# thierrydumas/autoencoder_based_image_compression

Hardware: AMD Instinct MI355X
Metric: Mpixels/s encode+decode (Kodak 768x512 luma), bitstream bit-exact (higher is better)
Workload: dtype f32; 1 GPU; kodak_512x768_luma_batch24_per_gpu_bin_width_1.0_lossless_roundtrip; height=512, width=768, truncated_unary_length=10, idx_map_exception=67, parallelism=single GPU, coder=device, 64 maps per wavefront, encode + decode + compare

## Files before the change

### autoencoder_based_image_compression_amd/csrc/hip/conv_gemm_split.hip

```cpp
#include "conv_gemm.h"

#include <cstdlib>

using namespace eae_conv_gemm;

namespace {

constexpr int RING = 8;
#ifndef EAE_EPI_RING
#define EAE_EPI_RING 4
#endif
constexpr int EPI_RING = EAE_EPI_RING;
constexpr int ABUF = 32 * AS_STRIDE;
constexpr int vec_floats(int norm) { return (norm >= NORM_LATENT ? 5 : 2) * EAE_C; }
constexpr int QT_H = 4, QT_W = 8;
constexpr int MIN_PIECE = 4;
constexpr int SPIN_LIMIT = 1 << 22;

__device__ __forceinline__ int head_steps(int d, int D, int T) {
    return T < 3 * MIN_PIECE ? T : MIN_PIECE + (d * (T - 2 * MIN_PIECE)) / D;
}

template <int NORM, int WPB>
__global__ __launch_bounds__(64 * WPB, NORM >= NORM_LATENT ? 2 : 3) void conv_gemm_split_kernel(const ConvGemmParams p) {
    __shared__ __attribute__((aligned(16))) float lds[WPB * 2 * ABUF + vec_floats(NORM)];
#ifdef EAE_GEMM_PRIO
    __builtin_amdgcn_s_setprio(EAE_GEMM_PRIO);
#endif
    const int lane = threadIdx.x & 63;
    const int wave = __builtin_amdgcn_readfirstlane(threadIdx.x >> 6);
    float* wlds = lds + wave * 2 * ABUF;
    float* vec_lds = lds + WPB * 2 * ABUF;
    {
        const float2 z = make_float2(0.f, 0.f);
        *reinterpret_cast<float2*>(vec_lds + 2 * lane) = p.bias ? *reinterpret_cast<const float2*>(p.bias + 2 * lane) : z;
        if (NORM == EAE_NORM_GDN || NORM == EAE_NORM_IGDN || NORM == NORM_LATENT)
            *reinterpret_cast<float2*>(vec_lds + EAE_C + 2 * lane) = *reinterpret_cast<const float2*>(p.beta + 2 * lane);
        if (NORM >= NORM_LATENT) {
            if (NORM == NORM_LATENT_PLAIN) *reinterpret_cast<float2*>(vec_lds + EAE_C + 2 * lane) = z;
            *reinterpret_cast<float2*>(vec_lds + 2 * EAE_C + 2 * lane) = NORM == NORM_LATENT ? *reinterpret_cast<const float2*>(p.beta_out + 2 * lane) : z;
            *reinterpret_cast<float2*>(vec_lds + 3 * EAE_C + 2 * lane) = p.map_mean ? *reinterpret_cast<const float2*>(p.map_mean + 2 * lane) : z;
            *reinterpret_cast<float2*>(vec_lds + 4 * EAE_C + 2 * lane) = *reinterpret_cast<const float2*>(p.bin_widths + 2 * lane);
        }
    }
    const int hi = lane >> 5, lj = lane & 31, a_q = lane & 7;
    const int cbase = 4 * hi;

    const int x = (int)blockIdx.x & 7;
    const int wx = p.split_resident_waves_per_xcd;
    const int nsp = p.n * p.tiles_r * p.tiles_c;
    const int q8 = nsp >> 3, r8 = nsp & 7;
    const int cnt_sp = q8 + (x < r8 ? 1 : 0);
    const int first_sp = x * q8 + (x < r8 ? x : r8);
    const int ntt = cnt_sp * p.n_phases;
    const int D = p.split ? (ntt < wx ? ntt : wx) : 0;
    const int F = ntt - D;
    const int n_items = 2 * D + F;
    unsigned int* flags = p.split_ws + 256 + x * 1024;

    const __amdgpu_buffer_rsrc_t w_rsrc = __builtin_amdgcn_make_buffer_rsrc(
        const_cast<float*>(p.w), 0, (int)((size_t)MAX_TAPS * EAE_C * EAE_C * sizeof(float)), 0x00020000);
    const int w_lane = (hi * EAE_C + lj * 4) * 4;
    const int a_off = lj * AS_STRIDE + hi * 16;

    {
        const int item = ((int)blockIdx.x >> 3) * WPB + wave;
        if (item >= n_items) return;
        int d = -1, tau;
        bool is_tail = false;
        if (item < D) { d = item; tau = ntt - D + d; }
        else if (item < D + F) { tau = item - D; }
        else { d = item - D - F; tau = ntt - D + d; is_tail = true; }
        int ph = 0, sp = tau;
        while (sp >= cnt_sp) { sp -= cnt_sp; ++ph; }
        const PhaseDesc& pd = p.phase[ph];
        const int ntaps = pd.ntaps;
        const int tap_of_lane = pd.tap[lane < MAX_TAPS ? lane : 0];
#define EAE_Q_TAP(ti_) __builtin_amdgcn_readlane(tap_of_lane, (ti_))
        const int T = (EAE_C / KC) * ntaps;
        int s0 = 0, s1 = T;
        if (d >= 0) {
            const int h = head_steps(d, D, T);
            if (is_tail) { if (h >= T) return; s0 = h; }
            else s1 = h;
        }
        int b = first_sp + sp;
        const int tc = b % p.tiles_c; b /= p.tiles_c;
        const int tr = b % p.tiles_r;
        const int img = b / p.tiles_r;

        int a_pr[4], a_pc[4], a_ok[4];
        const int a_m0 = 4 * ((lane >> 3) & 3) + 16 * (lane >> 5);
#pragma unroll
        for (int i = 0; i < 4; ++i) {
            const int m = a_m0 + i;
            a_pr[i] = tr * QT_H + m / QT_W;
            a_pc[i] = tc * QT_W + m % QT_W;
            a_ok[i] = (a_pr[i] < p.hp) & (a_pc[i] < p.wp);
        }
        const float* in_img = p.in + (size_t)img * p.hin * p.win * EAE_C;
        const __amdgpu_buffer_rsrc_t in_rsrc = __builtin_amdgcn_make_buffer_rsrc(
            const_cast<float*>(in_img), 0, (int)((size_t)p.hin * p.win * EAE_C * sizeof(float)), 0x00020000);
        const int pr = tr * QT_H + lj / QT_W, pc = tc * QT_W + lj % QT_W;
        const bool valid = pr < p.hp && pc < p.wp;
        float* out_img = p.out + (size_t)img * p.hout * p.wout * EAE_C;
        const int o_off = ((pr * p.out_stride + pd.out_a) * p.wout + (pc * p.out_stride + pd.out_b)) * EAE_C;
        float* o = out_img + o_off;
        const __amdgpu_buffer_rsrc_t out_rsrc = __builtin_amdgcn_make_buffer_rsrc(
            out_img, 0, (int)((size_t)p.hout * p.wout * EAE_C * sizeof(float)), 0x00020000);
        const int park = valid ? (o_off + cbase) * 4 : -1;

        float4 a_reg[4];
#define EAE_Q_PREFETCH_A(packed_, ci0_)                                                                              \
        {                                                                                                            \
            const int dr_ = ((packed_) & 0xFF) - 8, dc_ = (((packed_) >> 8) & 0xFF) - 8;                             \
            _Pragma("unroll") for (int i = 0; i < 4; ++i) {                                                          \
                const int r_ = a_pr[i] * p.in_stride + dr_;                                                          \
                const int c_ = a_pc[i] * p.in_stride + dc_;                                                          \
                const int ok_ = a_ok[i] & ((unsigned)r_ < (unsigned)p.hin) & ((unsigned)c_ < (unsigned)p.win);       \
                const int lin_ = ((r_ * p.win + c_) * EAE_C + (ci0_) + 4 * a_q) * 4;                                 \
                const u32x4 v_ = __builtin_amdgcn_raw_buffer_load_b128(in_rsrc, ok_ ? lin_ : -1, 0, 0);              \
                a_reg[i] = make_float4(__uint_as_float(v_.x), __uint_as_float(v_.y), __uint_as_float(v_.z),          \
                                       __uint_as_float(v_.w));                                                       \
            }                                                                                                        \
        }
#define EAE_Q_STAGE_A(buf_)                                                                                          \
        {                                                                                                            \
            _Pragma("unroll") for (int i = 0; i < 4; ++i) {                                                          \
                float* dst_ = wlds + (buf_) * ABUF + (a_m0 + i) * AS_STRIDE + 2 * a_q;                              \
                *reinterpret_cast<float2*>(dst_) = make_float2(a_reg[i].x, a_reg[i].z);                              \
                *reinterpret_cast<float2*>(dst_ + 16) = make_float2(a_reg[i].y, a_reg[i].w);                         \
            }                                                                                                        \
        }
#define EAE_Q_SLAB(ti_, ch_) ((((EAE_Q_TAP(ti_) >> 16) * EAE_C + (ch_) * KC) * EAE_C) * 4)
#define EAE_Q_W_LOAD(dst_, slab_, kk_)                                                                               \
        {                                                                                                            \
            const u32x4 v_ = __builtin_amdgcn_raw_buffer_load_b128(w_rsrc, w_lane + (kk_) * 2 * EAE_C * 4, (slab_), 0); \
            dst_ = make_float4(__uint_as_float(v_.x), __uint_as_float(v_.y), __uint_as_float(v_.z),                  \
                               __uint_as_float(v_.w));                                                               \
        }

        f32x16 acc[4];
        if (s0 == 0) {
#pragma unroll
            for (int t = 0; t < 4; ++t)
#pragma unroll
                for (int r = 0; r < 16; ++r) acc[t][r] = 0.f;
        } else {
            int gave_up = 0;
            if (lane == 0) {
                int spins = 0;
                while (__hip_atomic_load(flags + d, __ATOMIC_RELAXED, __HIP_MEMORY_SCOPE_AGENT) == 0u) {
                    __builtin_amdgcn_s_sleep(8);
                    if (++spins > p.split_spin_limit) { gave_up = 1; break; }
                }
            }
            if (__builtin_amdgcn_readfirstlane(gave_up)) {
                if (lane == 0) atomicAdd(p.split_ws + SPLIT_ERROR_WORD, 1u);
                return;
            }
            __builtin_amdgcn_wave_barrier();
            asm volatile("" ::: "memory");
#pragma unroll
            for (int t = 0; t < 4; ++t)
#pragma unroll
                for (int g = 0; g < 4; ++g) {
                    const u32x4 v = __builtin_amdgcn_raw_buffer_load_b128(out_rsrc, park, (32 * t + 8 * g) * 4, 16);
                    acc[t][4 * g + 0] = __uint_as_float(v.x); acc[t][4 * g + 1] = __uint_as_float(v.y);
                    acc[t][4 * g + 2] = __uint_as_float(v.z); acc[t][4 * g + 3] = __uint_as_float(v.w);
                }
            if (lane == 0) __hip_atomic_store(flags + d, 0u, __ATOMIC_RELAXED, __HIP_MEMORY_SCOPE_AGENT);
        }

        int tap_i = s0 % ntaps, chunk = s0 / ntaps;
        float4 ring[RING];
        {
            const int slab0 = EAE_Q_SLAB(tap_i, chunk);
#pragma unroll
            for (int i = 0; i < RING; ++i) EAE_Q_W_LOAD(ring[i], slab0, i)
        }
        EAE_Q_PREFETCH_A(EAE_Q_TAP(tap_i), chunk * KC)
        EAE_Q_STAGE_A(0)
        for (int step = s0; step < s1; ++step) {
            int nti = tap_i + 1, nch = chunk;
            if (nti == ntaps) { nti = 0; ++nch; }
            if (step + 1 >= s1) { nti = tap_i; nch = chunk; }
            const int slab_cur = EAE_Q_SLAB(tap_i, chunk);
            const int slab_nxt = EAE_Q_SLAB(nti, nch);
            EAE_Q_PREFETCH_A(EAE_Q_TAP(nti), nch * KC)
            const float4* a_rd = reinterpret_cast<const float4*>(wlds + ((step - s0) & 1) * ABUF + a_off);
            const float4 a0 = a_rd[0], a1 = a_rd[1], a2 = a_rd[2], a3 = a_rd[3];
            const float av[16] = {a0.x, a0.y, a0.z, a0.w, a1.x, a1.y, a1.z, a1.w, a2.x, a2.y, a2.z, a2.w, a3.x, a3.y, a3.z, a3.w};
            __builtin_amdgcn_sched_barrier(0);
#pragma unroll
            for (int kk = 0; kk < KC / 2; ++kk) {
                const float4 wq = ring[kk % RING];
                acc[0] = mfma32(wq.x, av[kk], acc[0]);
                acc[1] = mfma32(wq.y, av[kk], acc[1]);
                acc[2] = mfma32(wq.z, av[kk], acc[2]);
                acc[3] = mfma32(wq.w, av[kk], acc[3]);
                if (kk + RING < KC / 2) { EAE_Q_W_LOAD(ring[kk % RING], slab_cur, kk + RING) }
                else { EAE_Q_W_LOAD(ring[kk % RING], slab_nxt, kk + RING - KC / 2) }
                __builtin_amdgcn_sched_group_barrier(0x008, 4, 0);
                __builtin_amdgcn_sched_group_barrier(0x020, 1, 0);
            }
            __builtin_amdgcn_sched_barrier(0);
            EAE_Q_STAGE_A(((step - s0) + 1) & 1)
            tap_i = nti;
            chunk = nch;
        }

        if (s1 == T) {
            if constexpr (NORM >= NORM_LATENT) {
                if (p.bias) {
#pragma unroll
                    for (int t = 0; t < 4; ++t)
#pragma unroll
                        for (int g = 0; g < 4; ++g) {
                            const float4 bv = *reinterpret_cast<const float4*>(vec_lds + 32 * t + 8 * g + cbase);
                            acc[t][4 * g + 0] = acc[t][4 * g + 0] + bv.x;
                            acc[t][4 * g + 1] = acc[t][4 * g + 1] + bv.y;
                            acc[t][4 * g + 2] = acc[t][4 * g + 2] + bv.z;
                            acc[t][4 * g + 3] = acc[t][4 * g + 3] + bv.w;
                        }
                }
                wave_latent_body<NORM == NORM_LATENT, NORM == NORM_LATENT>(acc, vec_lds + EAE_C, p.gamma, p.gamma_out, p.latent, valid,
                                                                           (long)img, pr * p.wp + pc, p.hp * p.wp, lane);
            } else {
                wave_epilogue<NORM, EPI_RING>(acc, vec_lds, p.bias != nullptr, p.gamma, o, valid, lane);
            }
        } else {
#pragma unroll
            for (int t = 0; t < 4; ++t)
#pragma unroll
                for (int g = 0; g < 4; ++g) {
                    const u32x4 v = {__float_as_uint(acc[t][4 * g]), __float_as_uint(acc[t][4 * g + 1]),
                                     __float_as_uint(acc[t][4 * g + 2]), __float_as_uint(acc[t][4 * g + 3])};
                    __builtin_amdgcn_raw_buffer_store_b128(v, out_rsrc, park, (32 * t + 8 * g) * 4, 16);
                }
            asm volatile("s_waitcnt vmcnt(0)" ::: "memory");
            if (lane == 0 && !p.split_mute_heads) __hip_atomic_store(flags + d, 1u, __ATOMIC_RELAXED, __HIP_MEMORY_SCOPE_AGENT);
        }
#undef EAE_Q_PREFETCH_A
#undef EAE_Q_STAGE_A
#undef EAE_Q_SLAB
#undef EAE_Q_TAP
#undef EAE_Q_W_LOAD
    }
}

}

int eae_conv_gemm::launch_split(ConvGemmParams& p, hipStream_t stream, int cut) {
    const int cus = eae_compute_units();
    if (cus < 8 || (cus & 7)) return 1;
    p.tiles_r = (p.hp + QT_H - 1) / QT_H;
    p.tiles_c = (p.wp + QT_W - 1) / QT_W;
    const long nsp = (long)p.n * p.tiles_r * p.tiles_c;
    const long tiles = nsp * p.n_phases;
    const long simds = 4L * cus;
    long k = tiles / simds;
    if (k > 3) k = 3;
    if (k < 1) k = 1;
    const bool validated = eae_is_whole_mi355x();
    bool split = cut > 0;
    if (cut > 0) k = cut > 3 ? 3 : cut;
    if (cut < 0 && validated && p.split_ws && p.n_phases == 1 && tiles >= simds) {
        const long rounds = (tiles + simds - 1) / simds;
        split = (double)rounds * simds > 1.03 * (double)tiles || tiles >= 3 * simds;
    }
    if (split && !p.split_ws) return EAE_HIP_BAD_ARGUMENT;
    if (p.norm >= NORM_LATENT && k > 2) k = 2;
    if ((cus / 8) * 4 * k > 1024) return 1;
    for (int i = 1; i < p.n_phases; ++i)
        for (int j = i; j > 0 && p.phase[j].ntaps > p.phase[j - 1].ntaps; --j) {
            const PhaseDesc tmp = p.phase[j]; p.phase[j] = p.phase[j - 1]; p.phase[j - 1] = tmp;
        }
    p.split = split ? 1 : 0;
    p.split_spin_limit = SPIN_LIMIT;
    p.split_mute_heads = 0;
    if (split) {
        if (g_eae_launch_options.split_mute) { p.split_mute_heads = 1; p.split_spin_limit = 1 << 12; }
    }
    p.split_resident_waves_per_xcd = (cus / 8) * 4 * (int)k;
    const long cnt_max = (nsp + 7) / 8 * p.n_phases;
    const long d_max = split ? (cnt_max < p.split_resident_waves_per_xcd ? cnt_max : p.split_resident_waves_per_xcd) : 0;
    const int wpb = g_eae_launch_options.split_wpb == 1 ? 1 : 4;
    const int grid = (int)((cnt_max + d_max + wpb - 1) / wpb) * 8;
#define EAE_LAUNCH_S(N_)                                                                                                  \
    {                                                                                                                     \
        if (wpb == 1) hipLaunchKernelGGL((conv_gemm_split_kernel<N_, 1>), dim3(grid), dim3(64), 0, stream, p);            \
        else hipLaunchKernelGGL((conv_gemm_split_kernel<N_, 4>), dim3(grid), dim3(256), 0, stream, p);                    \
    }
    if (p.norm == NORM_LATENT) EAE_LAUNCH_S(NORM_LATENT)
    else if (p.norm == NORM_LATENT_PLAIN) EAE_LAUNCH_S(NORM_LATENT_PLAIN)
    else if (p.norm == EAE_NORM_GDN) EAE_LAUNCH_S(EAE_NORM_GDN)
    else if (p.norm == EAE_NORM_IGDN) EAE_LAUNCH_S(EAE_NORM_IGDN)
    else EAE_LAUNCH_S(EAE_NORM_NONE)
#undef EAE_LAUNCH_S
    EAE_HIP_CHECK_LAUNCH();
    return EAE_HIP_OK;
}
```

Measured before the change: 2976 Mpixels/s.

## Simplify A-tile staging with padded single LDS buffer and precomputed tap masks

Replaces the double-buffered, swizzled A-tile LDS staging with one buffer per wave using a KC+1 padded row stride. Each lane now loads its own output pixel's channels, and the per-element LDS reads are stride-2. Address math is simplified: a per-lane base offset plus a bitmask of out-of-bounds taps, computed once per work item, replace the per-prefetch row/column bounds checks. The aims are to cut VALU address arithmetic and LDS footprint. The cost is 16 scalar LDS reads and scalar writes per step instead of vector ones, and reliance on in-order LDS access within a wave for the single buffer.

Measured after the change: 3026 Mpixels/s, median of 6. +1.7%, better.

```diff
diff --git a/autoencoder_based_image_compression_amd/csrc/hip/conv_gemm_split.hip b/autoencoder_based_image_compression_amd/csrc/hip/conv_gemm_split.hip
--- a/autoencoder_based_image_compression_amd/csrc/hip/conv_gemm_split.hip
+++ b/autoencoder_based_image_compression_amd/csrc/hip/conv_gemm_split.hip
@@ -11,7 +11,8 @@
 #define EAE_EPI_RING 4
 #endif
 constexpr int EPI_RING = EAE_EPI_RING;
-constexpr int ABUF = 32 * AS_STRIDE;
+constexpr int A_STRIDE = KC + 1;
+constexpr int ABUF = 32 * A_STRIDE;
 constexpr int vec_floats(int norm) { return (norm >= NORM_LATENT ? 5 : 2) * EAE_C; }
 constexpr int QT_H = 4, QT_W = 8;
 constexpr int MIN_PIECE = 4;
@@ -23,14 +24,14 @@
 
 template <int NORM, int WPB>
 __global__ __launch_bounds__(64 * WPB, NORM >= NORM_LATENT ? 2 : 3) void conv_gemm_split_kernel(const ConvGemmParams p) {
-    __shared__ __attribute__((aligned(16))) float lds[WPB * 2 * ABUF + vec_floats(NORM)];
+    __shared__ __attribute__((aligned(16))) float lds[WPB * ABUF + vec_floats(NORM)];
 #ifdef EAE_GEMM_PRIO
     __builtin_amdgcn_s_setprio(EAE_GEMM_PRIO);
 #endif
     const int lane = threadIdx.x & 63;
     const int wave = __builtin_amdgcn_readfirstlane(threadIdx.x >> 6);
-    float* wlds = lds + wave * 2 * ABUF;
-    float* vec_lds = lds + WPB * 2 * ABUF;
+    float* wlds = lds + wave * ABUF;
+    float* vec_lds = lds + WPB * ABUF;
     {
         const float2 z = make_float2(0.f, 0.f);
         *reinterpret_cast<float2*>(vec_lds + 2 * lane) = p.bias ? *reinterpret_cast<const float2*>(p.bias + 2 * lane) : z;
@@ -43,7 +44,7 @@
             *reinterpret_cast<float2*>(vec_lds + 4 * EAE_C + 2 * lane) = *reinterpret_cast<const float2*>(p.bin_widths + 2 * lane);
         }
     }
-    const int hi = lane >> 5, lj = lane & 31, a_q = lane & 7;
+    const int hi = lane >> 5, lj = lane & 31;
     const int cbase = 4 * hi;
 
     const int x = (int)blockIdx.x & 7;
@@ -61,7 +62,6 @@
     const __amdgpu_buffer_rsrc_t w_rsrc = __builtin_amdgcn_make_buffer_rsrc(
         const_cast<float*>(p.w), 0, (int)((size_t)MAX_TAPS * EAE_C * EAE_C * sizeof(float)), 0x00020000);
     const int w_lane = (hi * EAE_C + lj * 4) * 4;
-    const int a_off = lj * AS_STRIDE + hi * 16;
 
     {
         const int item = ((int)blockIdx.x >> 3) * WPB + wave;
@@ -89,18 +89,6 @@
         const int tr = b % p.tiles_r;
         const int img = b / p.tiles_r;
 
-        int a_pr[4], a_pc[4], a_ok[4];
-        const int a_m0 = 4 * ((lane >> 3) & 3) + 16 * (lane >> 5);
-#pragma unroll
-        for (int i = 0; i < 4; ++i) {
-            const int m = a_m0 + i;
-            a_pr[i] = tr * QT_H + m / QT_W;
-            a_pc[i] = tc * QT_W + m % QT_W;
-            a_ok[i] = (a_pr[i] < p.hp) & (a_pc[i] < p.wp);
-        }
-        const float* in_img = p.in + (size_t)img * p.hin * p.win * EAE_C;
-        const __amdgpu_buffer_rsrc_t in_rsrc = __builtin_amdgcn_make_buffer_rsrc(
-            const_cast<float*>(in_img), 0, (int)((size_t)p.hin * p.win * EAE_C * sizeof(float)), 0x00020000);
         const int pr = tr * QT_H + lj / QT_W, pc = tc * QT_W + lj % QT_W;
         const bool valid = pr < p.hp && pc < p.wp;
         float* out_img = p.out + (size_t)img * p.hout * p.wout * EAE_C;
@@ -110,29 +98,38 @@
             out_img, 0, (int)((size_t)p.hout * p.wout * EAE_C * sizeof(float)), 0x00020000);
         const int park = valid ? (o_off + cbase) * 4 : -1;
 
+        const float* in_img = p.in + (size_t)img * p.hin * p.win * EAE_C;
+        const __amdgpu_buffer_rsrc_t in_rsrc = __builtin_amdgcn_make_buffer_rsrc(
+            const_cast<float*>(in_img), 0, (int)((size_t)p.hin * p.win * EAE_C * sizeof(float)), 0x00020000);
+        const int a_r = pr * p.in_stride, a_c = pc * p.in_stride;
+        const unsigned int a_base = ((unsigned)a_r * (unsigned)p.win + (unsigned)a_c) * (EAE_C * 4) + 16 * hi;
+        unsigned int a_inv = 0;
+        for (int ti = 0; ti < ntaps; ++ti) {
+            const int packed = EAE_Q_TAP(ti);
+            const int r = a_r + (packed & 0xFF) - 8, c = a_c + ((packed >> 8) & 0xFF) - 8;
+            if (!valid || (unsigned)r >= (unsigned)p.hin || (unsigned)c >= (unsigned)p.win) a_inv |= 1u << ti;
+        }
+
         float4 a_reg[4];
-#define EAE_Q_PREFETCH_A(packed_, ci0_)                                                                              \
+#define EAE_Q_PREFETCH_A(packed_, ti_, ci0_)                                                                         \
         {                                                                                                            \
             const int dr_ = ((packed_) & 0xFF) - 8, dc_ = (((packed_) >> 8) & 0xFF) - 8;                             \
+            const unsigned int off_ = (a_base + (unsigned)(((dr_ * p.win + dc_) * EAE_C + (ci0_)) * 4)) |            \
+                                      ((a_inv >> (ti_)) << 31);                                                      \
             _Pragma("unroll") for (int i = 0; i < 4; ++i) {                                                          \
-                const int r_ = a_pr[i] * p.in_stride + dr_;                                                          \
-                const int c_ = a_pc[i] * p.in_stride + dc_;                                                          \
-                const int ok_ = a_ok[i] & ((unsigned)r_ < (unsigned)p.hin) & ((unsigned)c_ < (unsigned)p.win);       \
-                const int lin_ = ((r_ * p.win + c_) * EAE_C + (ci0_) + 4 * a_q) * 4;                                 \
-                const u32x4 v_ = __builtin_amdgcn_raw_buffer_load_b128(in_rsrc, ok_ ? lin_ : -1, 0, 0);              \
+                const u32x4 v_ = __builtin_amdgcn_raw_buffer_load_b128(in_rsrc, (int)off_ + 32 * i, 0, 0);           \
                 a_reg[i] = make_float4(__uint_as_float(v_.x), __uint_as_float(v_.y), __uint_as_float(v_.z),          \
                                        __uint_as_float(v_.w));                                                       \
             }                                                                                                        \
         }
-#define EAE_Q_STAGE_A(buf_)                                                                                          \
+#define EAE_Q_STAGE_A()                                                                                              \
         {                                                                                                            \
             _Pragma("unroll") for (int i = 0; i < 4; ++i) {                                                          \
-                float* dst_ = wlds + (buf_) * ABUF + (a_m0 + i) * AS_STRIDE + 2 * a_q;                              \
-                *reinterpret_cast<float2*>(dst_) = make_float2(a_reg[i].x, a_reg[i].z);                              \
-                *reinterpret_cast<float2*>(dst_ + 16) = make_float2(a_reg[i].y, a_reg[i].w);                         \
+                float* dst_ = wlds + lj * A_STRIDE + 8 * i + 4 * hi;                                                 \
+                dst_[0] = a_reg[i].x; dst_[1] = a_reg[i].y; dst_[2] = a_reg[i].z; dst_[3] = a_reg[i].w;              \
             }                                                                                                        \
         }
-#define EAE_Q_SLAB(ti_, ch_) ((((EAE_Q_TAP(ti_) >> 16) * EAE_C + (ch_) * KC) * EAE_C) * 4)
+#define EAE_Q_SLAB(packed_, ch_) (((((packed_) >> 16) * EAE_C + (ch_) * KC) * EAE_C) * 4)
 #define EAE_Q_W_LOAD(dst_, slab_, kk_)                                                                               \
         {                                                                                                            \
             const u32x4 v_ = __builtin_amdgcn_raw_buffer_load_b128(w_rsrc, w_lane + (kk_) * 2 * EAE_C * 4, (slab_), 0); \
@@ -173,24 +170,27 @@
         }
 
         int tap_i = s0 % ntaps, chunk = s0 / ntaps;
+        int tap_cur = EAE_Q_TAP(tap_i);
         float4 ring[RING];
         {
-            const int slab0 = EAE_Q_SLAB(tap_i, chunk);
+            const int slab0 = EAE_Q_SLAB(tap_cur, chunk);
 #pragma unroll
             for (int i = 0; i < RING; ++i) EAE_Q_W_LOAD(ring[i], slab0, i)
         }
-        EAE_Q_PREFETCH_A(EAE_Q_TAP(tap_i), chunk * KC)
-        EAE_Q_STAGE_A(0)
+        EAE_Q_PREFETCH_A(tap_cur, tap_i, chunk * KC)
+        EAE_Q_STAGE_A()
+        const float* a_rd = wlds + lj * A_STRIDE + hi;
         for (int step = s0; step < s1; ++step) {
             int nti = tap_i + 1, nch = chunk;
             if (nti == ntaps) { nti = 0; ++nch; }
             if (step + 1 >= s1) { nti = tap_i; nch = chunk; }
-            const int slab_cur = EAE_Q_SLAB(tap_i, chunk);
-            const int slab_nxt = EAE_Q_SLAB(nti, nch);
-            EAE_Q_PREFETCH_A(EAE_Q_TAP(nti), nch * KC)
-            const float4* a_rd = reinterpret_cast<const float4*>(wlds + ((step - s0) & 1) * ABUF + a_off);
-            const float4 a0 = a_rd[0], a1 = a_rd[1], a2 = a_rd[2], a3 = a_rd[3];
-            const float av[16] = {a0.x, a0.y, a0.z, a0.w, a1.x, a1.y, a1.z, a1.w, a2.x, a2.y, a2.z, a2.w, a3.x, a3.y, a3.z, a3.w};
+            const int tap_nxt = EAE_Q_TAP(nti);
+            const int slab_cur = EAE_Q_SLAB(tap_cur, chunk);
+            const int slab_nxt = EAE_Q_SLAB(tap_nxt, nch);
+            EAE_Q_PREFETCH_A(tap_nxt, nti, nch * KC)
+            float av[16];
+#pragma unroll
+            for (int kk = 0; kk < KC / 2; ++kk) av[kk] = a_rd[2 * kk];
             __builtin_amdgcn_sched_barrier(0);
 #pragma unroll
             for (int kk = 0; kk < KC / 2; ++kk) {
@@ -205,9 +205,10 @@
                 __builtin_amdgcn_sched_group_barrier(0x020, 1, 0);
             }
             __builtin_amdgcn_sched_barrier(0);
-            EAE_Q_STAGE_A(((step - s0) + 1) & 1)
+            EAE_Q_STAGE_A()
             tap_i = nti;
             chunk = nch;
+            tap_cur = tap_nxt;
         }
 
         if (s1 == T) {
```
